# prs-eth/ResDepth

Hardware: AMD Instinct MI355X
Metric: DSM tiles/sec fwd+bwd (256x256, 3-ch, depth-5 U-Net) (higher is better)
Workload: dtype f32

## Files before the change

resdepth_amd/csrc/rd_common.h:

```cpp
#pragma once
#include <hip/hip_runtime.h>
#include <stdint.h>
#include <stdio.h>

#include <tuple>
#include <utility>

#include "../../include/resdepth_hip.h"

namespace rd {

void set_error(const char* fmt, ...);
int check_hip(hipError_t e, const char* what);

struct QuantArgs;
int prof_level();
void prof_begin(hipStream_t s, const char* cls, double flops, double bytes);
void prof_end(hipStream_t s);

struct ProfScope {
    hipStream_t s;
    bool on;
    ProfScope(hipStream_t s_, const char* cls, double flops, double bytes, bool mfma_class = false)
        : s(s_), on(prof_level() >= (mfma_class ? 1 : 2)) {
        if (on) prof_begin(s, cls, flops, bytes);
    }
    ~ProfScope() {
        if (on) prof_end(s);
    }
};

int bn_reduce_finalize(const float* partial, int nb, int c, double count, float eps, float momentum, float* mean, float* invstd,
                       float* rmean, float* rvar, int64_t* nbt, hipStream_t s);
int reduce_partials_f32(const float* partial, double* sums, int nb, int qc, hipStream_t s);

enum TuneKey {
    TUNE_MFMA_F32 = 0,
    TUNE_NT_TILE,
    TUNE_NT_HALO,
    TUNE_NT_SKEW,
    TUNE_TN_TILE,
    TUNE_TN_BLOCKS,
    TUNE_TN_SPLIT,
    TUNE_WG_STRIP,
    TUNE_WG_MINBLOCKS,
    TUNE_WG_BLOCKS,
    TUNE_WG_OCC,
    TUNE_CONVT_PATCH,
    TUNE_EDGE_CONV,
    TUNE_ROWS_BLOCKS,
    TUNE_LAST_BLOCKS,
    TUNE_NT_SPLITK,
    TUNE_NT_EPI,
    TUNE_MFMA_PRODUCTS,
    TUNE_D2H_BLOCKS,
    TUNE_COUNT
};
int tune(int key);
inline int mfma_split() { return !tune(TUNE_MFMA_F32); }
inline int mfma_products() { return tune(TUNE_MFMA_PRODUCTS) == 3 ? 3 : 6; }
struct QuantArgs {
    const unsigned* a;
    const unsigned* b;
    unsigned* out;
    unsigned* out2;
    int img_stride;
};
QuantArgs quant_take();
QuantArgs quant_take_img();
int wgrad_strip_splits(int n, int h, int w, int cin, int cout);
int wgrad_strip_launch(const float* x, const float* dz, float* slab, int n, int h, int w, int cin, int cout, hipStream_t s,
                       int* splits_out, int* swapped_out, const unsigned* x_amax = nullptr, const unsigned* dz_amax = nullptr);

int convt_fwd_launch(const float* x, const void* wsplit, size_t wsplit_bytes, const float* bias, const float* skip,
                     const float* sk_mean, const float* sk_invstd, const float* sk_gamma, const float* sk_beta, float sk_slope,
                     const float* sk_slope_dev, float* out, int n, int h, int w, int cin, int cout, hipStream_t s, int* launched,
                     const QuantArgs& qa);

size_t convt_wgrad_ws_bytes(int n, int h, int w, int cin, int cout);
int convt_wgrad_launch(const float* x, const float* dout, float* slab, int n, int h, int w, int cin, int cout, hipStream_t s,
                       int* splits_out, const unsigned* x_amax = nullptr, const unsigned* dout_amax = nullptr);

int conv_last_fwd_launch(const float* s_in, const float* wt, const float* bias, const float* x_nchw, int xc, float* out, int n,
                         int h, int w, int c, hipStream_t s, int* launched);
int conv_last_dgrad_launch(const float* dout, const float* wt, float* ds, int n, int h, int w, int c, hipStream_t s, int* launched);
int conv_last_dgrad_bn_launch(const float* dout, const float* wt, float* ds, int n, int h, int w, int c, const float* bn_z,
                              const float* mean, const float* invstd, const float* gamma, const float* beta, float slope,
                              const float* slope_dev, float* part, hipStream_t s, int* rows);
int conv_last_wgrad_blocks(int n, int h, int w, int c);
struct TailSkip {
    const float* z;
    const float* mean;
    const float* invstd;
    const float* gamma;
    const float* beta;
    const float* slope_dev;
    float slope;
};
int tail_compose_launch(const float* wt, const float* bt, const float* wl, float* M, float* V, float* VT, float* B9, int cin, int c0,
                        hipStream_t s);
int conv_last_fwd_tail_launch(const TailSkip& sk, const float* t16, const float* b9, const float* wt, const float* bias,
                              const float* x_nchw, int xc, float* out, int n, int h, int w, int c, hipStream_t s);
int conv_last_wgrad_tail_launch(const TailSkip& sk, const float* dout, double* partial, int n, int h, int w, int c, hipStream_t s);
int tail_t16_launch(const TailSkip& sk, const float* V, float* t16, long pixels, int cin, hipStream_t s);
int convt_last_wgrad_launch(const float* x, const TailSkip& sk, const float* dout, const float* wl, float* dwt, double* partial,
                            double* c16, int n, int hc, int wc, int cin, int c0, hipStream_t s);
int conv_last_tail_blocks(int n, int h, int w);
long edge_tiles(int n, int h, int w);
// ... 186 lines not shown
```

resdepth_amd/csrc/rd_elementwise.hip:

```cpp
#include <stdlib.h>

#include "rd_common.h"
#include "rd_mfma_dev.h"

namespace rd {

static inline int grid_cap(long g, int cap) {
    if (g > cap) g = cap;
    if (g < 1) g = 1;
    return (int)g;
}

__device__ __forceinline__ float act_fn(float y, float slope) { return y > 0.f ? y : y * slope; }
__device__ __forceinline__ float act_grad(float y, float slope) { return y > 0.f ? 1.f : slope; }

template <int K>
__device__ __forceinline__ void reduce_rows(double (&vals)[K], double* red, int t, int CQ, int RP, bool active) {
#pragma unroll
    for (int k = 0; k < K; ++k) red[k * 256 + t] = active ? vals[k] : 0.0;
    __syncthreads();
    if (t < CQ) {
#pragma unroll
        for (int k = 0; k < K; ++k) {
            double s = 0.0;
// ... 231 lines not shown
        if (sidx == 2 && dextra) dextra[c] = (float)r;
    }
}

__global__ __launch_bounds__(512) void bn_reduce_finalize_quad_kernel(const float* __restrict__ partial, int nb, int C, double count,
                                                                      float eps, float momentum, float* __restrict__ mean,
                                                                      float* __restrict__ invstd, float* __restrict__ rmean,
                                                                      float* __restrict__ rvar, int64_t* nbt) {
    __shared__ double red[512][4];
    const int t = threadIdx.x, kind = t & 1, slice = t >> 1, cq = blockIdx.x;
    const float* base = partial + (long)kind * C + cq * 4;
    const long stride = 2L * C;
    double a0 = 0.0, a1 = 0.0, a2 = 0.0, a3 = 0.0;
    int b = slice;
    for (; b + 7 * 256 < nb; b += 8 * 256) {
        float4 v[8];
#pragma unroll
        for (int k = 0; k < 8; ++k) v[k] = *reinterpret_cast<const float4*>(base + (long)(b + 256 * k) * stride);
#pragma unroll
        for (int k = 0; k < 8; ++k) {
            a0 += v[k].x; a1 += v[k].y; a2 += v[k].z; a3 += v[k].w;
        }
    }
    for (; b < nb; b += 256) {
        const float4 v = *reinterpret_cast<const float4*>(base + (long)b * stride);
        a0 += v.x; a1 += v.y; a2 += v.z; a3 += v.w;
    }
    red[t][0] = a0; red[t][1] = a1; red[t][2] = a2; red[t][3] = a3;
    __syncthreads();
    for (int sl = 128; sl >= 1; sl >>= 1) {
        if (slice < sl) {
#pragma unroll
            for (int k = 0; k < 4; ++k) red[t][k] += red[t + 2 * sl][k];
        }
        __syncthreads();
    }
    if (t == 0 && blockIdx.x == 0 && nbt) *nbt += 1;
    if (t < 4) {
        const int c = cq * 4 + t;
        const double su = red[0][t], sq = red[1][t];
        const double m = su / count;
        double var = sq / count - m * m;
        if (var < 0.0) var = 0.0;
        mean[c] = (float)m;
        invstd[c] = (float)(1.0 / sqrt(var + (double)eps));
        if (rmean) rmean[c] = (1.f - momentum) * rmean[c] + momentum * (float)m;
        if (rvar) {
            const double unb = count > 1.0 ? var * count / (count - 1.0) : var;
            rvar[c] = (1.f - momentum) * rvar[c] + momentum * (float)unb;
        }
    }
}

int bn_reduce_finalize(const float* partial, int nb, int c, double count, float eps, float momentum, float* mean, float* invstd,
                       float* rmean, float* rvar, int64_t* nbt, hipStream_t s) {
    if (c % 4 == 0)
        RD_LAUNCH(bn_reduce_finalize_quad_kernel, dim3(c / 4), dim3(512), 0, s, partial, nb, c, count, eps, momentum, mean,
                           invstd, rmean, rvar, nbt);
    else
        RD_LAUNCH(bn_reduce_finalize_kernel, dim3(cdiv(c, 4)), dim3(256), 0, s, partial, nb, c, count, eps, momentum, mean,
                           invstd, rmean, rvar, nbt);
    RD_LAUNCH_CHECK("bn_reduce_finalize");
    return RD_OK;
}

__global__ void bn_eval_stats_kernel(const float* __restrict__ rmean, const float* __restrict__ rvar, float eps,
                                     float* __restrict__ mean, float* __restrict__ invstd, int C) {
    const int c = blockIdx.x * blockDim.x + threadIdx.x;
    if (c >= C) return;
    mean[c] = rmean[c];
    invstd[c] = 1.f / sqrtf(rvar[c] + eps);
}

template <bool POOL>
__global__ __launch_bounds__(256) void bn_act_pool_fwd_kernel(const float* __restrict__ z, const float* __restrict__ mean,
                                                              const float* __restrict__ invstd,
                                                              const float* __restrict__ gamma,
                                                              const float* __restrict__ beta, float slope_val,
                                                              const float* __restrict__ slope_dev,
                                                              float* __restrict__ a, float* __restrict__ pooled,
                                                              uint8_t* __restrict__ idx, float* __restrict__ zpool, long rows,
                                                              int H, int W, int C, int CQ, unsigned* a_amax, unsigned* p_amax) {
    const float slope = slope_dev ? slope_dev[0] : slope_val;
    const long total = rows * CQ;
    float amx = 0.f, pmx = 0.f;
    long e0, e1;
    block_range(total, blockIdx.x, gridDim.x, blockDim.x, e0, e1);
    for (long e = e0 + threadIdx.x; e < e1; e += blockDim.x) {
        const int cq = (int)(e % CQ);
        const long row = e / CQ;
        const float4 mu = *reinterpret_cast<const float4*>(mean + cq * 4);
        const float4 is = *reinterpret_cast<const float4*>(invstd + cq * 4);
        const float4 ga = *reinterpret_cast<const float4*>(gamma + cq * 4);
        const float4 be = *reinterpret_cast<const float4*>(beta + cq * 4);
        const float sc[4] = {is.x * ga.x, is.y * ga.y, is.z * ga.z, is.w * ga.w};
        const float sh[4] = {be.x - mu.x * sc[0], be.y - mu.y * sc[1], be.z - mu.z * sc[2], be.w - mu.w * sc[3]};
        if (!POOL) {
            const float4 x = ld_nt4(z + row * C + cq * 4);
            float4 y;
            y.x = act_fn(fmaf(x.x, sc[0], sh[0]), slope);
            y.y = act_fn(fmaf(x.y, sc[1], sh[1]), slope);
            y.z = act_fn(fmaf(x.z, sc[2], sh[2]), slope);
            y.w = act_fn(fmaf(x.w, sc[3], sh[3]), slope);
            *reinterpret_cast<float4*>(a + row * C + cq * 4) = y;
            amx = amax_acc(amax_acc(amax_acc(amax_acc(amx, y.x), y.y), y.z), y.w);
        } else {
            const int W2 = W >> 1, H2 = H >> 1;
            const int j = (int)(row % W2);
            const int i = (int)((row / W2) % H2);
// ... 388 lines not shown
                const float sv[4] = {s4[u].x, s4[u].y, s4[u].z, s4[u].w};
#pragma unroll
                for (int tap = 0; tap < 9; ++tap) {
                    const int dy = tap / 3 - 1, dx = tap % 3 - 1;
                    const int sy = yy - dy, sx = xx - dx;
                    float d = 0.f;
                    if ((unsigned)sy < uH && (unsigned)sx < uW) d = dout[p - dy * W - dx];
#pragma unroll
                    for (int k = 0; k < 4; ++k) acc[tap][k] = fmaf(sv[k], d, acc[tap][k]);
                    if (tap == 4 && cq == 0) accb += d;
                }
            }
        }
    }
    double* out = partial + (long)blockIdx.x * (9 * C + 1);
#pragma unroll
    for (int tap = 0; tap < 9; ++tap) {
        double v[4];
#pragma unroll
        for (int k = 0; k < 4; ++k) v[k] = acc[tap][k];
        reduce_rows<4>(v, red, t, CQ, RP, active);
        if (t < CQ) {
#pragma unroll
            for (int k = 0; k < 4; ++k) out[tap * C + cq * 4 + k] = v[k];
        }
    }
    double vb[4] = {(double)accb, 0.0, 0.0, 0.0};
    reduce_rows<4>(vb, red, t, CQ, RP, active);
    if (t == 0) out[9 * C] = vb[0];
}

__global__ __launch_bounds__(256) void last_wgrad_reduce_kernel(const double* __restrict__ partial,
                                                                float* __restrict__ dw, float* __restrict__ dbias,
                                                                int nb, int C) {
    __shared__ double red[256];
    const int tot = 9 * C + 1;
    const double r = sliced_column_sum<double>(partial, nb, tot, tot, red);
    const int e = blockIdx.x * 16 + threadIdx.x;
    if (threadIdx.x < 16 && e < tot) {
        if (e == 9 * C) {
            if (dbias) dbias[0] = (float)r;
        } else {
            const int tap = e / C, ci = e % C;
            dw[ci * 9 + tap] = (float)r;
        }
    }
}

__device__ __forceinline__ float denorm(float v, float sd, float mu) { return __fadd_rn(__fmul_rn(v, sd), mu); }

__global__ __launch_bounds__(256) void l1_partial_kernel(const float* __restrict__ yp, const float* __restrict__ y,
                                                         const uint8_t* __restrict__ mask, const float* __restrict__ mean,
                                                         const float* __restrict__ stdv, double* __restrict__ partial,
                                                         long total, long pps) {
    __shared__ double red[2 * 256];
    double s = 0.0, c = 0.0;
    for (long e = (long)blockIdx.x * blockDim.x + threadIdx.x; e < total; e += (long)gridDim.x * blockDim.x) {
        if (mask[e]) {
            const int n = (int)(e / pps);
            const float sd = stdv[n], mu = mean[n];
            s += (double)fabsf(denorm(yp[e], sd, mu) - denorm(y[e], sd, mu));
            c += 1.0;
        }
    }
    red[threadIdx.x] = s;
    red[256 + threadIdx.x] = c;
    __syncthreads();
    for (int off = 128; off > 0; off >>= 1) {
        if ((int)threadIdx.x < off) {
            red[threadIdx.x] += red[threadIdx.x + off];
            red[256 + threadIdx.x] += red[256 + threadIdx.x + off];
        }
        __syncthreads();
    }
    if (threadIdx.x == 0) {
        partial[blockIdx.x * 2] = red[0];
        partial[blockIdx.x * 2 + 1] = red[256];
    }
}

__global__ __launch_bounds__(256) void l1_reduce_kernel(const double* __restrict__ partial, double* __restrict__ sums,
                                                        int nb) {
    __shared__ double red[2 * 256];
    double s = 0.0, c = 0.0;
    for (int b = threadIdx.x; b < nb; b += 256) {
        s += partial[b * 2];
        c += partial[b * 2 + 1];
    }
    red[threadIdx.x] = s;
    red[256 + threadIdx.x] = c;
    __syncthreads();
    for (int off = 128; off > 0; off >>= 1) {
        if ((int)threadIdx.x < off) {
            red[threadIdx.x] += red[threadIdx.x + off];
            red[256 + threadIdx.x] += red[256 + threadIdx.x + off];
        }
        __syncthreads();
    }
    if (threadIdx.x == 0) {
        sums[0] = red[0];
        sums[1] = red[256];
    }
}

__global__ __launch_bounds__(256) void l1_finish_kernel(const float* __restrict__ yp, const float* __restrict__ y,
                                                        const uint8_t* __restrict__ mask, const float* __restrict__ mean,
                                                        const float* __restrict__ stdv, const double* __restrict__ sums,
                                                        double numel_total, const float* __restrict__ gout_dev,
                                                        float* __restrict__ loss, float* __restrict__ dyp, long total,
                                                        long pps) {
    const float cnt = (float)sums[1], numel = (float)numel_total;
    const float gout = gout_dev ? gout_dev[0] : 1.f;
    if (blockIdx.x == 0 && threadIdx.x == 0 && loss) {
        float l = (float)(sums[0] / numel_total);
        l = l * numel;
        loss[0] = l / cnt;
    }
    if (!dyp) return;
    const float g = ((gout / cnt) * numel) / numel;
    for (long e = (long)blockIdx.x * blockDim.x + threadIdx.x; e < total; e += (long)gridDim.x * blockDim.x) {
        float o = 0.f;
        if (mask[e]) {
            const int n = (int)(e / pps);
            const float sd = stdv[n], mu = mean[n];
            const float d = denorm(yp[e], sd, mu) - denorm(y[e], sd, mu);
            const float sg = d > 0.f ? 1.f : (d < 0.f ? -1.f : 0.f);
            o = g * sg * sd;
        }
        dyp[e] = o;
    }
// ... 695 lines not shown
    } else {
        ProfScope ps((hipStream_t)s, "bn_act_fwd", 0, 8.0 * pixels * c);
        RD_LAUNCH((bn_act_pool_fwd_kernel<false>), dim3(grid_cap((pixels * CQ + 255) / 256, 8192)), dim3(256),
                           0, (hipStream_t)s, z, mean, invstd, gamma, beta, slope, slope_dev, a, (float*)nullptr,
                           (uint8_t*)nullptr, (float*)nullptr, pixels, h, w, c, CQ, qa.out, (unsigned*)nullptr);
    }
    RD_LAUNCH_CHECK("bn_act_pool_fwd");
    return RD_OK;
}

size_t rd_bn_act_bwd_ws_bytes(int n, int h, int w, int c) {
    RowPlan pl;
    if (!plan_rows((long)n * h * w, c, &pl)) return 0;
    return (size_t)pl.nb * 4 * c * sizeof(double);
}

int rd_bn_act_bwd_reduce(const float* z, const float* mean, const float* invstd, const float* gamma, const float* beta,
                         float slope, const float* slope_dev, const float* g_full, const float* g_pool,
                         const uint8_t* idx, double* sums, float* dgamma, float* dbeta, float* dextra, int n, int h, int w, int c,
                         void* ws, size_t ws_bytes, rd_stream_t s) {
    RD_REQUIRE(z && mean && invstd && gamma && beta && sums, "rd_bn_act_bwd_reduce: null pointer");
    RD_REQUIRE(g_full || g_pool, "rd_bn_act_bwd_reduce: no gradient source");
    RD_REQUIRE(!g_pool || idx, "rd_bn_act_bwd_reduce: g_pool needs idx");
    const bool pool = g_pool != nullptr;
    const long pixels = (long)n * h * w;
    const long rows = pool ? pixels / 4 : pixels;
    RowPlan pl;
    RD_REQUIRE(plan_rows(rows, c, &pl), "rd_bn_act_bwd_reduce: C must be a multiple of 4 and <= 1024 (got %d)", c);
    size_t need = (size_t)pl.nb * 4 * c * sizeof(double);
    if (const size_t q = rd_bn_act_bwd_ws_bytes(n, h, w, c); q > need) need = q;
    if (!ws || ws_bytes < need) {
        set_error("rd_bn_act_bwd_reduce: workspace too small (%zu < %zu)", ws_bytes, need);
        return RD_ERR_WS;
    }
    ProfScope ps((hipStream_t)s, "bn_act_bwd_reduce", 0, 4.0 * pixels * c * (1 + (g_full ? 1 : 0) + (pool ? 0.3 : 0)));
    if (pool)
        RD_LAUNCH((bn_act_bwd_kernel<true, false>), dim3(pl.nb), dim3(256), 0, (hipStream_t)s, z, mean, invstd,
                           gamma, beta, slope, slope_dev, g_full, g_pool, idx, (double*)ws, (const double*)nullptr, 1.0, 1,
                           (float*)nullptr, rows, h, w, c, pl.CQ, pl.RP, pl.rows_per_block, (unsigned*)nullptr);
    else
        RD_LAUNCH((bn_act_bwd_kernel<false, false>), dim3(pl.nb), dim3(256), 0, (hipStream_t)s, z, mean,
                           invstd, gamma, beta, slope, slope_dev, g_full, g_pool, idx, (double*)ws, (const double*)nullptr, 1.0, 1,
                           (float*)nullptr, rows, h, w, c, pl.CQ, pl.RP, pl.rows_per_block, (unsigned*)nullptr);
    RD_LAUNCH(partial_reduce_kernel, dim3(cdiv(4 * c, 16)), dim3(256), 0, (hipStream_t)s, (const double*)ws,
                       sums, pl.nb, 4 * c, c, dbeta, dgamma, dextra);
    RD_LAUNCH_CHECK("bn_act_bwd_reduce");
    return RD_OK;
}

int rd_bn_bwd_stats_finalize(const float* part_a, int rows_a, const float* part_b, int rows_b, int c, double* sums,
                             float* dgamma, float* dbeta, float* dextra, rd_stream_t s) {
    RD_REQUIRE(part_a && rows_a > 0 && sums && c > 0 && c % 4 == 0 && (!part_b || rows_b > 0), "rd_bn_bwd_stats_finalize: bad arguments");
    ProfScope ps((hipStream_t)s, "bn_act_bwd_reduce", 0, 16.0 * c * ((double)rows_a + (part_b ? rows_b : 0)));
    RD_LAUNCH(bn_bwd_stats_finalize_kernel, dim3(c), dim3(256), 0, (hipStream_t)s, part_a, rows_a, part_b,
                       part_b ? rows_b : 0, c, sums, dgamma, dbeta, dextra);
    RD_LAUNCH_CHECK("bn_bwd_stats_finalize");
    return RD_OK;
}

int rd_bn_act_bwd_apply(const float* z, const float* mean, const float* invstd, const float* gamma, const float* beta,
                        float slope, const float* slope_dev, const float* g_full, const float* g_pool,
                        const uint8_t* idx, const double* sums,
                        double count, int training, float* dz, float* dgamma, float* dbeta, int n, int h, int w, int c,
                        rd_stream_t s) {
    RD_REQUIRE(z && mean && invstd && gamma && beta && sums && dz, "rd_bn_act_bwd_apply: null pointer");
    RD_REQUIRE(g_full || g_pool, "rd_bn_act_bwd_apply: no gradient source");
    RD_REQUIRE(!g_pool || idx, "rd_bn_act_bwd_apply: g_pool needs idx");
    RD_REQUIRE(count > 0, "rd_bn_act_bwd_apply: count must be positive");
    const QuantArgs qa = quant_take();
    const bool pool = g_pool != nullptr;
    const long pixels = (long)n * h * w;
    const long rows = pool ? pixels / 4 : pixels;
    RowPlan pl;
    RD_REQUIRE(plan_rows(rows, c, &pl), "rd_bn_act_bwd_apply: C must be a multiple of 4 and <= 1024 (got %d)", c);
    {
        ProfScope ps((hipStream_t)s, "bn_act_bwd_apply", 0,
                     4.0 * pixels * c * (2 + (g_full ? 1 : 0) + (pool ? 0.3 : 0)));
        if (pool)
            RD_LAUNCH((bn_act_bwd_kernel<true, true>), dim3(pl.nb), dim3(256), 0, (hipStream_t)s, z, mean,
                               invstd, gamma, beta, slope, slope_dev, g_full, g_pool, idx, (double*)nullptr, sums, count,
                               training, dz, rows, h, w, c, pl.CQ, pl.RP, pl.rows_per_block, qa.out);
        else
            RD_LAUNCH((bn_act_bwd_kernel<false, true>), dim3(pl.nb), dim3(256), 0, (hipStream_t)s, z, mean,
                               invstd, gamma, beta, slope, slope_dev, g_full, g_pool, idx, (double*)nullptr, sums, count, training,
                               dz, rows, h, w, c, pl.CQ, pl.RP, pl.rows_per_block, qa.out);
    }
    if (dgamma || dbeta)
        RD_LAUNCH(bn_param_grad_kernel, dim3(cdiv(c, 256)), dim3(256), 0, (hipStream_t)s, sums, dgamma, dbeta,
                           c);
    RD_LAUNCH_CHECK("bn_act_bwd_apply");
    return RD_OK;
}

}

static int first_grid(int n, int h, int w, int* tiles_x, int* tiles_y, int* ntiles) {
    *tiles_x = cdiv(w, FT_W);
    *tiles_y = cdiv(h, FT_H);
    *ntiles = n * (*tiles_x) * (*tiles_y);
    return *ntiles < 512 ? *ntiles : 512;
}

template <bool WGRAD>
static int launch_first(const float* x, const float* wt, float* z, const float* dz, float* partial, int n, int h, int w,
                        int cin, int cout, int grid, int tiles_x, int tiles_y, int ntiles, hipStream_t s) {
    const int CQ = cout / 4, PS = 256 / CQ;
#define RD_FIRST_CASE(CI)                                                                                              \
    case CI:                                                                                                           \
// ... 356 lines not shown
    ProfScope ps((hipStream_t)s, "convt_last_wgrad", 2.0 * n * hc * wc * 16.0 * cin, 4.0 * n * hc * wc * (double)(cin + 4));
    const TailSkip sk = {x, mean, invstd, gamma, beta, slope_dev, slope};
    return convt_last_wgrad_launch(x, sk, dout, w_last, dwt_iohw, partial, c16, n, hc, wc, cin, c0, (hipStream_t)s);
}

size_t rd_conv3x3_last_bwd_weight_ws_bytes(int n, int h, int w, int c) {
    if (const int nb = conv_last_wgrad_blocks(n, h, w, c)) return (size_t)nb * (9 * c + 1) * sizeof(double);
    RowPlan pl;
    if (!plan_rows((long)n * h * w, c, &pl, last_blocks())) return 0;
    return (size_t)pl.nb * (9 * c + 1) * sizeof(double);
}

int rd_conv3x3_last_bwd_weight(const float* s_in, const float* dout, float* dw, float* dbias, int n, int h, int w,
                               int c, void* ws, size_t ws_bytes, rd_stream_t s) {
    RD_REQUIRE(s_in && dout && dw, "rd_conv3x3_last_bwd_weight: null pointer");
    RowPlan pl;
    RD_REQUIRE(plan_rows((long)n * h * w, c, &pl, last_blocks()), "rd_conv3x3_last_bwd_weight: C must be a multiple of 4, <= 1024");
    RD_REQUIRE((long)n * h * w < (1L << 31), "rd_conv3x3_last_bwd_weight: pixel count must be < 2^31");
    const size_t need = rd_conv3x3_last_bwd_weight_ws_bytes(n, h, w, c);
    if (!ws || ws_bytes < need) {
        set_error("rd_conv3x3_last_bwd_weight: workspace too small (%zu < %zu)", ws_bytes, need);
        return RD_ERR_WS;
    }
    ProfScope ps((hipStream_t)s, "conv_last_wgrad", 2.0 * n * h * w * 9.0 * c, 4.0 * n * h * w * (double)(c + 1));
    if (const int nb = conv_last_wgrad_blocks(n, h, w, c)) {
        if (int e = conv_last_wgrad_launch(s_in, dout, (double*)ws, n, h, w, c, (hipStream_t)s)) return e;
        RD_LAUNCH(last_wgrad_reduce_kernel, dim3(cdiv(9 * c + 1, 16)), dim3(256), 0, (hipStream_t)s,
                           (const double*)ws, dw, dbias, nb, c);
        RD_LAUNCH_CHECK("conv_last_wgrad");
        return RD_OK;
    }
    RD_LAUNCH(conv_last_wgrad_kernel, dim3(pl.nb), dim3(256), 0, (hipStream_t)s, s_in, dout, (double*)ws,
                       (long)n * h * w, h, w, c, pl.CQ, pl.RP, pl.rows_per_block);
    RD_LAUNCH(last_wgrad_reduce_kernel, dim3(cdiv(9 * c + 1, 16)), dim3(256), 0, (hipStream_t)s,
                       (const double*)ws, dw, dbias, pl.nb, c);
    RD_LAUNCH_CHECK("conv_last_wgrad");
    return RD_OK;
}

static int l1_grid(long total) { return grid_cap((total + 255) / 256, 1024); }

size_t rd_masked_l1_ws_bytes(long long numel) { return (size_t)l1_grid(numel) * 2 * sizeof(double); }

int rd_masked_l1_partial(const float* yp, const float* y, const uint8_t* mask, const float* mean, const float* stdv,
                         double* sums, int n, long long pps, void* ws, size_t ws_bytes, rd_stream_t s) {
    RD_REQUIRE(yp && y && mask && mean && stdv && sums && n > 0 && pps > 0, "rd_masked_l1_partial: bad arguments");
    const long total = (long)n * pps;
    const int nb = l1_grid(total);
    if (!ws || ws_bytes < (size_t)nb * 2 * sizeof(double)) {
        set_error("rd_masked_l1_partial: workspace too small");
        return RD_ERR_WS;
    }
    ProfScope ps((hipStream_t)s, "masked_l1", 0, 9.0 * total);
    RD_LAUNCH(l1_partial_kernel, dim3(nb), dim3(256), 0, (hipStream_t)s, yp, y, mask, mean, stdv, (double*)ws,
                       total, (long)pps);
    RD_LAUNCH(l1_reduce_kernel, dim3(1), dim3(256), 0, (hipStream_t)s, (const double*)ws, sums, nb);
    RD_LAUNCH_CHECK("masked_l1_partial");
    return RD_OK;
}

int rd_masked_l1_finish(const float* yp, const float* y, const uint8_t* mask, const float* mean, const float* stdv,
                        const double* sums, double numel_total, const float* gout, float* loss, float* dyp, int n,
                        long long pps, rd_stream_t s) {
    RD_REQUIRE(yp && y && mask && mean && stdv && sums && n > 0 && pps > 0, "rd_masked_l1_finish: bad arguments");
    const long total = (long)n * pps;
    ProfScope ps((hipStream_t)s, "masked_l1", 0, 13.0 * total);
    RD_LAUNCH(l1_finish_kernel, dim3(dyp ? l1_grid(total) : 1), dim3(256), 0, (hipStream_t)s, yp, y, mask, mean,
                       stdv, sums, numel_total, gout, loss, dyp, total, (long)pps);
    RD_LAUNCH_CHECK("masked_l1_finish");
    return RD_OK;
}

int rd_adam_step(float* p, const float* g, float* m, float* v, long long numel, double beta1, double beta2, float eps,
                 float weight_decay, float step_size, float bc2_sqrt, float grad_scale, rd_stream_t s) {
    RD_REQUIRE(p && g && m && v && numel > 0, "rd_adam_step: bad arguments");
    ProfScope ps((hipStream_t)s, "adam", 0, 28.0 * numel);
    RD_LAUNCH(adam_kernel, dim3(grid_cap((numel + 255) / 256, 8192)), dim3(256), 0, (hipStream_t)s, p, g, m, v,
                       (long)numel, (float)(1.0 - beta1), (float)beta2, (float)(1.0 - beta2), eps, weight_decay, step_size, bc2_sqrt,
                       grad_scale);
    RD_LAUNCH_CHECK("adam");
    return RD_OK;
}

int rd_adam_step_dev(float* p, const float* g, float* m, float* v, long long numel, const float* scalars_dev, rd_stream_t s) {
    RD_REQUIRE(p && g && m && v && scalars_dev && numel > 0, "rd_adam_step_dev: bad arguments");
    ProfScope ps((hipStream_t)s, "adam", 0, 28.0 * numel);
    RD_LAUNCH(adam_dev_kernel, dim3(grid_cap((numel + 255) / 256, 8192)), dim3(256), 0, (hipStream_t)s, p, g, m, v,
                       (long)numel, scalars_dev);
    RD_LAUNCH_CHECK("adam_dev");
    return RD_OK;
}

int rd_sgd_step(float* p, const float* g, float* momentum_buf, long long numel, float lr, float weight_decay, float momentum,
                float dampening, int nesterov, int first_step, float grad_scale, rd_stream_t s) {
    RD_REQUIRE(p && g && numel > 0, "rd_sgd_step: bad arguments");
    RD_REQUIRE(momentum == 0.f || momentum_buf, "rd_sgd_step: momentum != 0 needs a momentum buffer");
    ProfScope ps((hipStream_t)s, "sgd", 0, (momentum != 0.f ? 20.0 : 12.0) * numel);
    const dim3 grid(grid_cap((numel + 255) / 256, 8192));
    if (momentum != 0.f)
        RD_LAUNCH(sgd_kernel<true>, grid, dim3(256), 0, (hipStream_t)s, p, g, momentum_buf, (long)numel, lr, weight_decay,
                           momentum, 1.f - dampening, nesterov, first_step, grad_scale);
    else
        RD_LAUNCH(sgd_kernel<false>, grid, dim3(256), 0, (hipStream_t)s, p, g, (float*)nullptr, (long)numel, lr,
                           weight_decay, 0.f, 1.f, 0, 0, grad_scale);
    RD_LAUNCH_CHECK("sgd");
    return RD_OK;
}

int rd_blend_accumulate(const float* pred, const float* mean, const float* stdv, const int* pos, const int* reg, int n,
// ... 197 lines not shown
```

resdepth_amd/csrc/rd_runtime.hip:

```cpp
#include <hip/hip_ext.h>
#include <stdarg.h>
#include <stdlib.h>
#include <string.h>

#include <mutex>
#include <string>
#include <vector>

#include "rd_common.h"

namespace rd {

static thread_local char g_err[512] = "";

static void quant_clear();
void set_error(const char* fmt, ...) {
    quant_clear();
    va_list ap;
    va_start(ap, fmt);
    vsnprintf(g_err, sizeof(g_err), fmt, ap);
    va_end(ap);
}

int check_hip(hipError_t e, const char* what) {
    if (e == hipSuccess) return RD_OK;
    set_error("%s: %s", what, hipGetErrorString(e));
    return RD_ERR_HIP;
}

struct TuneEntry {
    const char* name;
    int value;
};
static TuneEntry g_tune[TUNE_COUNT] = {
    {"mfma_f32", 0},   {"nt_tile", -1},      {"nt_halo", -1},    {"nt_skew", 1},     {"tn_tile", -1},     {"tn_blocks", 512}, {"tn_split", -1},
    {"wg_strip", -1},  {"wg_minblocks", 768}, {"wg_blocks", 512}, {"wg_occ", 2}, {"convt_patch", -1}, {"edge_conv", -1}, {"rows_blocks", 512}, {"last_blocks", 2048},
    {"nt_splitk", -1}, {"nt_epi", -1}, {"mfma_products", 3}, {"d2h_blocks", 0},
};
static int tune_index(const char* name, size_t len) {
    for (int i = 0; i < TUNE_COUNT; ++i)
        if (strlen(g_tune[i].name) == len && !strncmp(g_tune[i].name, name, len)) return i;
    return -1;
}
static const int g_tune_env = [] {
    if (const char* m = getenv("RD_MFMA"))
    {
        if (!strcmp(m, "f32")) g_tune[TUNE_MFMA_F32].value = 1;
        if (!strcmp(m, "split2h")) g_tune[TUNE_MFMA_PRODUCTS].value = 3;
        if (!strcmp(m, "split3")) g_tune[TUNE_MFMA_PRODUCTS].value = 6;
    }
    const char* e = getenv("RD_TUNE");
    while (e && *e) {
        const char* eq = strchr(e, '=');
        if (!eq) break;
        const int i = tune_index(e, (size_t)(eq - e));
        if (i >= 0) g_tune[i].value = atoi(eq + 1);
        e = strchr(eq, ',');
        if (e) ++e;
    }
    return 0;
}();
int tune(int key) { return g_tune[key].value; }

static thread_local QuantArgs t_quant = {nullptr, nullptr, nullptr, nullptr, 0};
static void quant_clear() { t_quant = {nullptr, nullptr, nullptr, nullptr, 0}; }
QuantArgs quant_take_img() {
    const QuantArgs q = t_quant;
    t_quant = {nullptr, nullptr, nullptr, nullptr, 0};
    return q;
}
QuantArgs quant_take() {
    QuantArgs q = t_quant;
    t_quant = {nullptr, nullptr, nullptr, nullptr, 0};
    if (q.img_stride) q = {nullptr, nullptr, nullptr, nullptr, 0};
    return q;
}

struct PlanOp {
    int kind;
    int role;
    const void* fn;
    dim3 grid, block;
    unsigned shmem;
    int nargs;
    size_t arg0;
    int ev;
};
struct Plan {
    std::vector<PlanOp> ops;
    std::vector<size_t> arg_off;
// ... 102 lines not shown
}

void prof_begin(hipStream_t s, const char* cls, double flops, double bytes) {
    std::lock_guard<std::mutex> lk(g_mu);
    int ci = -1;
    for (size_t i = 0; i < g_cls.size(); ++i)
        if (g_cls[i].name == cls) ci = (int)i;
    if (ci < 0) {
        if (g_cls.size() >= RD_PROF_MAX_CLASSES) return;
        g_cls.push_back(ProfClass());
        g_cls.back().name = cls;
        ci = (int)g_cls.size() - 1;
    }
    ProfRec r;
    r.cls = ci;
    r.e0 = get_event();
    r.e1 = get_event();
    r.flops = flops;
    r.bytes = bytes;
    if (!r.e0 || !r.e1) return;
    (void)hipEventRecord(r.e0, s);
    g_recs.push_back(r);
    t_open = (int)g_recs.size() - 1;
}

void prof_end(hipStream_t s) {
    std::lock_guard<std::mutex> lk(g_mu);
    if (t_open < 0 || t_open >= (int)g_recs.size()) return;
    (void)hipEventRecord(g_recs[t_open].e1, s);
    t_open = -1;
}

static void drain_locked() {
    for (auto& r : g_recs) {
        (void)hipEventSynchronize(r.e1);
        float ms = 0.f;
        if (hipEventElapsedTime(&ms, r.e0, r.e1) == hipSuccess) {
            ProfClass& c = g_cls[r.cls];
            c.launches += 1;
            c.ms += ms;
            c.flops += r.flops;
            c.bytes += r.bytes;
        }
        g_free_events.push_back(r.e0);
        g_free_events.push_back(r.e1);
    }
    g_recs.clear();
}

}

extern "C" {

int rd_version(void) { return 112; }

const char* rd_last_error_string(void) { return rd::g_err; }

int rd_plan_begin(rd_stream_t main_stream, rd_stream_t side_stream) {
    using namespace rd;
    std::lock_guard<std::mutex> lk(g_plan_mu);
    if (g_rec) {
        set_error("rd_plan_begin: a plan is already being recorded");
        return RD_ERR_ARG;
    }
    Plan* p = new Plan();
    p->rec[0] = (hipStream_t)main_stream;
    p->rec[1] = (hipStream_t)side_stream;
    (void)hipGetDevice(&p->dev);
    g_rec = p;
    g_recording = 1;
    return RD_OK;
}

int rd_plan_event_record(rd_stream_t stream) {
    using namespace rd;
    std::lock_guard<std::mutex> lk(g_plan_mu);
    if (!g_rec) return -1;
    const int role = plan_role(g_rec, (hipStream_t)stream);
    if (role < 0) return -1;
    PlanOp op = {};
    op.kind = 1; op.role = role; op.ev = g_rec->n_events++;
    g_rec->ops.push_back(op);
    return op.ev;
}

int rd_plan_event_wait(rd_stream_t stream, int ev) {
    using namespace rd;
    std::lock_guard<std::mutex> lk(g_plan_mu);
    if (!g_rec) return RD_OK;
    const int role = plan_role(g_rec, (hipStream_t)stream);
    if (role < 0 || ev < 0) {
        if (role >= 0 && !g_rec->poisoned) {
            g_rec->poisoned = true;
            g_rec->why = "a plan stream waited for an event recorded outside the plan";
        }
        return RD_OK;
    }
    PlanOp op = {};
    op.kind = 2; op.role = role; op.ev = ev;
    g_rec->ops.push_back(op);
    return RD_OK;
}

int rd_plan_segment(void) {
    using namespace rd;
    std::lock_guard<std::mutex> lk(g_plan_mu);
    if (!g_rec) return -1;
// ... 285 lines not shown
```

Measured before the change: 4514.

## Split BN finalize reductions across blocks with last-block tickets; fuse L1 reduce

Adds multi-block versions of the BatchNorm forward-stats finalize and backward-stats finalize kernels. Each channel quad's partial-sum reduction is spread over 32 or 16 blocks, with partials published to a workspace slab and an atomic ticket electing the last block to combine them. The masked-L1 loss now does its final reduction inside the partial kernel using a two-level ticket scheme, which removes the separate single-block reduce launch. This targets the poor parallelism of one-block-per-channel finalize kernels on large partial counts. In exchange it adds atomic and ticket traffic and depends on shared split-k workspace tickets that must be reset correctly.

```diff
diff --git a/resdepth_amd/csrc/rd_common.h b/resdepth_amd/csrc/rd_common.h
--- a/resdepth_amd/csrc/rd_common.h
+++ b/resdepth_amd/csrc/rd_common.h
@@ -54,6 +54,9 @@
     TUNE_NT_EPI,
     TUNE_MFMA_PRODUCTS,
     TUNE_D2H_BLOCKS,
+    TUNE_BN_FIN_SPLIT,
+    TUNE_BN_BWD_FIN_SPLIT,
+    TUNE_L1_FUSED,
     TUNE_COUNT
 };
 int tune(int key);
diff --git a/resdepth_amd/csrc/rd_elementwise.hip b/resdepth_amd/csrc/rd_elementwise.hip
--- a/resdepth_amd/csrc/rd_elementwise.hip
+++ b/resdepth_amd/csrc/rd_elementwise.hip
@@ -307,9 +307,192 @@
     }
 }
 
+constexpr int kTicketPitch = 32;
+constexpr int kFinTicketLines = 448;
+__device__ __forceinline__ bool last_block_of(unsigned* ticket, unsigned blocks, int* flag) {
+    __atomic_signal_fence(__ATOMIC_SEQ_CST);
+    __builtin_amdgcn_s_waitcnt(0x0F70);
+    __syncthreads();
+    if (threadIdx.x == 0) {
+        const unsigned prev = __hip_atomic_fetch_add(ticket, 1u, __ATOMIC_RELAXED, __HIP_MEMORY_SCOPE_AGENT);
+        *flag = prev == blocks - 1;
+        if (*flag) __hip_atomic_store(ticket, 0u, __ATOMIC_RELAXED, __HIP_MEMORY_SCOPE_AGENT);
+    }
+    __syncthreads();
+    __atomic_signal_fence(__ATOMIC_SEQ_CST);
+    return *flag != 0;
+}
+
+constexpr int kFinBlocks = 32;
+__global__ __launch_bounds__(128) void bn_reduce_finalize_quad_mb_kernel(const float* __restrict__ partial, int nb, int C, double count,
+                                                                         float eps, float momentum, float* __restrict__ mean,
+                                                                         float* __restrict__ invstd, float* __restrict__ rmean,
+                                                                         float* __restrict__ rvar, int64_t* nbt, double* pub,
+                                                                         unsigned* tickets) {
+    __shared__ float4 stage[16][65];
+    __shared__ double red[16][4];
+    __shared__ int last;
+    const int t = threadIdx.x, cq = blockIdx.x / kFinBlocks, r = blockIdx.x - cq * kFinBlocks;
+    const int lp = t & 15, lj = t >> 4;
+    const int lslice = r + 32 * (lp >> 1);
+    const int lrows = lslice < nb ? (nb - lslice + 255) >> 8 : 0;
+    const float* base = partial + (long)(lp & 1) * C + cq * 4 + (long)lslice * 2 * C;
+    const long stride = 512L * C;
+    const int ap = t >> 2, ak = t & 3;
+    const int aslice = r + 32 * (ap >> 1);
+    const int arows = (t < 64 && aslice < nb) ? (nb - aslice + 255) >> 8 : 0;
+    const int rows_max = r < nb ? (nb - r + 255) >> 8 : 0;
+    double acc = 0.0;
+    for (int i0 = 0; i0 < rows_max; i0 += 64) {
+        float4 v[8];
+#pragma unroll
+        for (int k = 0; k < 8; ++k) {
+            const int i = i0 + lj + 8 * k;
+            v[k] = i < lrows ? *reinterpret_cast<const float4*>(base + (long)i * stride) : make_float4(0.f, 0.f, 0.f, 0.f);
+        }
+#pragma unroll
+        for (int k = 0; k < 8; ++k) stage[lp][lj + 8 * k] = v[k];
+        __syncthreads();
+        const int cnt = arows - i0 < 64 ? arows - i0 : 64;
+        for (int i = 0; i < cnt; ++i) acc += reinterpret_cast<const float*>(&stage[ap][i])[ak];
+        __syncthreads();
+    }
+    if (t < 64) red[ap][ak] = acc;
+    __syncthreads();
+    const int kind = (t >> 2) & 1;
+    if (t < 8) {
+        const double l0 = red[0 + kind][ak] + red[8 + kind][ak], l1 = red[2 + kind][ak] + red[10 + kind][ak];
+        const double l2 = red[4 + kind][ak] + red[12 + kind][ak], l3 = red[6 + kind][ak] + red[14 + kind][ak];
+        const double root = (l0 + l2) + (l1 + l3);
+        __hip_atomic_store(pub + (((long)cq * kFinBlocks + r) * 2 + kind) * 4 + ak, root, __ATOMIC_RELAXED, __HIP_MEMORY_SCOPE_AGENT);
+    }
+    if (!last_block_of(tickets + cq * kTicketPitch, kFinBlocks, &last)) return;
+    if (t < 8) {
+        double x[kFinBlocks];
+#pragma unroll
+        for (int i = 0; i < kFinBlocks; ++i)
+            x[i] = __hip_atomic_load(pub + (((long)cq * kFinBlocks + i) * 2 + kind) * 4 + ak, __ATOMIC_RELAXED, __HIP_MEMORY_SCOPE_AGENT);
+#pragma unroll
+        for (int sl = 16; sl >= 1; sl >>= 1)
+#pragma unroll
+            for (int i = 0; i < sl; ++i) x[i] += x[i + sl];
+        red[kind][ak] = x[0];
+    }
+    __syncthreads();
+    if (t == 0 && cq == 0 && nbt) *nbt += 1;
+    if (t < 4) {
+        const int c = cq * 4 + t;
+        const double su = red[0][t], sq = red[1][t];
+        const double m = su / count;
+        double var = sq / count - m * m;
+        if (var < 0.0) var = 0.0;
+        mean[c] = (float)m;
+        invstd[c] = (float)(1.0 / sqrt(var + (double)eps));
+        if (rmean) rmean[c] = (1.f - momentum) * rmean[c] + momentum * (float)m;
+        if (rvar) {
+            const double unb = count > 1.0 ? var * count / (count - 1.0) : var;
+            rvar[c] = (1.f - momentum) * rvar[c] + momentum * (float)unb;
+        }
+    }
+}
+
+constexpr int kBwdFinBlocks = 16;
+__global__ __launch_bounds__(64) void bn_bwd_stats_finalize_mb_kernel(const float* __restrict__ pa, int ra, const float* __restrict__ pb,
+                                                                      int rb, int C, double* __restrict__ sums,
+                                                                      float* __restrict__ dgamma, float* __restrict__ dbeta,
+                                                                      float* __restrict__ dextra, double* pub, unsigned* tickets) {
+    __shared__ int last;
+    const int t = threadIdx.x, sidx = t & 3, sl = t >> 2;
+    const int cq = blockIdx.x / kBwdFinBlocks, j = blockIdx.x - cq * kBwdFinBlocks;
+    const long col = (long)sidx * C + cq * 4, stride = 4L * C;
+    double a0 = 0.0, a1 = 0.0, a2 = 0.0, a3 = 0.0;
+    for (int src = 0; src < 2; ++src) {
+        const float* part = src ? pb : pa;
+        const int nb = src ? rb : ra;
+        if (!part) continue;
+        int b = j * 16 + sl;
+        for (; b + 15 * 256 < nb; b += 16 * 256) {
+            float4 v[16];
+#pragma unroll
+            for (int k = 0; k < 16; ++k) v[k] = *reinterpret_cast<const float4*>(part + (long)(b + 256 * k) * stride + col);
+#pragma unroll
+            for (int k = 0; k < 16; k += 4) {
+                a0 += ((double)v[k].x + (double)v[k + 1].x) + ((double)v[k + 2].x + (double)v[k + 3].x);
+                a1 += ((double)v[k].y + (double)v[k + 1].y) + ((double)v[k + 2].y + (double)v[k + 3].y);
+                a2 += ((double)v[k].z + (double)v[k + 1].z) + ((double)v[k + 2].z + (double)v[k + 3].z);
+                a3 += ((double)v[k].w + (double)v[k + 1].w) + ((double)v[k + 2].w + (double)v[k + 3].w);
+            }
+        }
+        for (; b + 768 < nb; b += 1024) {
+            const float4 v0 = *reinterpret_cast<const float4*>(part + (long)b * stride + col);
+            const float4 v1 = *reinterpret_cast<const float4*>(part + (long)(b + 256) * stride + col);
+            const float4 v2 = *reinterpret_cast<const float4*>(part + (long)(b + 512) * stride + col);
+            const float4 v3 = *reinterpret_cast<const float4*>(part + (long)(b + 768) * stride + col);
+            a0 += ((double)v0.x + (double)v1.x) + ((double)v2.x + (double)v3.x);
+            a1 += ((double)v0.y + (double)v1.y) + ((double)v2.y + (double)v3.y);
+            a2 += ((double)v0.z + (double)v1.z) + ((double)v2.z + (double)v3.z);
+            a3 += ((double)v0.w + (double)v1.w) + ((double)v2.w + (double)v3.w);
+        }
+        for (; b < nb; b += 256) {
+            const float4 v = *reinterpret_cast<const float4*>(part + (long)b * stride + col);
+            a0 += v.x; a1 += v.y; a2 += v.z; a3 += v.w;
+        }
+    }
+#pragma unroll
+    for (int o = 4; o < 64; o <<= 1) {
+        a0 += __shfl_xor(a0, o);
+        a1 += __shfl_xor(a1, o);
+        a2 += __shfl_xor(a2, o);
+        a3 += __shfl_xor(a3, o);
+    }
+    if (t < 4) {
+        double* mine = pub + (((long)cq * kBwdFinBlocks + j) * 4 + sidx) * 4;
+        __hip_atomic_store(mine + 0, a0, __ATOMIC_RELAXED, __HIP_MEMORY_SCOPE_AGENT);
+        __hip_atomic_store(mine + 1, a1, __ATOMIC_RELAXED, __HIP_MEMORY_SCOPE_AGENT);
+        __hip_atomic_store(mine + 2, a2, __ATOMIC_RELAXED, __HIP_MEMORY_SCOPE_AGENT);
+        __hip_atomic_store(mine + 3, a3, __ATOMIC_RELAXED, __HIP_MEMORY_SCOPE_AGENT);
+    }
+    if (!last_block_of(tickets + cq * kTicketPitch, kBwdFinBlocks, &last)) return;
+    if (t < 16) {
+        const int si = t >> 2, k = t & 3;
+        double w[4];
+#pragma unroll
+        for (int wv = 0; wv < 4; ++wv) {
+            double x[4];
+#pragma unroll
+            for (int i = 0; i < 4; ++i)
+                x[i] = __hip_atomic_load(pub + (((long)cq * kBwdFinBlocks + wv * 4 + i) * 4 + si) * 4 + k, __ATOMIC_RELAXED,
+                                         __HIP_MEMORY_SCOPE_AGENT);
+            w[wv] = (x[0] + x[1]) + (x[2] + x[3]);
+        }
+        const double r = ((w[0] + w[1]) + w[2]) + w[3];
+        const int c = cq * 4 + k;
+        sums[(long)si * C + c] = r;
+        if (si == 0 && dbeta) dbeta[c] = (float)r;
+        if (si == 1 && dgamma) dgamma[c] = (float)r;
+        if (si == 2 && dextra) dextra[c] = (float)r;
+    }
+}
+
+static bool finalize_scratch(hipStream_t s, int c, double** pub, unsigned** tickets) {
+    int n_tickets = 0;
+    float* slab = nullptr;
+    size_t slab_bytes = 0;
+    if (!splitk_workspace(s, tickets, &n_tickets, &slab, &slab_bytes)) return false;
+    *pub = reinterpret_cast<double*>(slab);
+    return c / 4 <= kFinTicketLines && (kFinTicketLines + 33) * kTicketPitch <= n_tickets && (size_t)c * 512 <= slab_bytes;
+}
+
 int bn_reduce_finalize(const float* partial, int nb, int c, double count, float eps, float momentum, float* mean, float* invstd,
                        float* rmean, float* rvar, int64_t* nbt, hipStream_t s) {
-    if (c % 4 == 0)
+    const int split = tune(TUNE_BN_FIN_SPLIT);
+    double* pub = nullptr;
+    unsigned* tickets = nullptr;
+    const bool many = split > 0 && (nb >= split || (2L * nb >= split && (long)nb * c >= 128L * split));
+    if (c % 4 == 0 && many && finalize_scratch(s, c, &pub, &tickets))
+        RD_LAUNCH(bn_reduce_finalize_quad_mb_kernel, dim3(c / 4 * kFinBlocks), dim3(128), 0, s, partial, nb, c, count, eps, momentum,
+                           mean, invstd, rmean, rvar, nbt, pub, tickets);
+    else if (c % 4 == 0)
         RD_LAUNCH(bn_reduce_finalize_quad_kernel, dim3(c / 4), dim3(512), 0, s, partial, nb, c, count, eps, momentum, mean,
                            invstd, rmean, rvar, nbt);
     else
@@ -804,8 +987,10 @@
 __global__ __launch_bounds__(256) void l1_partial_kernel(const float* __restrict__ yp, const float* __restrict__ y,
                                                          const uint8_t* __restrict__ mask, const float* __restrict__ mean,
                                                          const float* __restrict__ stdv, double* __restrict__ partial,
-                                                         long total, long pps) {
+                                                         long total, long pps, double* __restrict__ sums,
+                                                         unsigned* ticket) {
     __shared__ double red[2 * 256];
+    __shared__ int last;
     double s = 0.0, c = 0.0;
     for (long e = (long)blockIdx.x * blockDim.x + threadIdx.x; e < total; e += (long)gridDim.x * blockDim.x) {
         if (mask[e]) {
@@ -825,9 +1010,39 @@
         }
         __syncthreads();
     }
+    if (!ticket) {
+        if (threadIdx.x == 0) {
+            partial[blockIdx.x * 2] = red[0];
+            partial[blockIdx.x * 2 + 1] = red[256];
+        }
+        return;
+    }
     if (threadIdx.x == 0) {
-        partial[blockIdx.x * 2] = red[0];
-        partial[blockIdx.x * 2 + 1] = red[256];
+        __hip_atomic_store(partial + blockIdx.x * 2, red[0], __ATOMIC_RELAXED, __HIP_MEMORY_SCOPE_AGENT);
+        __hip_atomic_store(partial + blockIdx.x * 2 + 1, red[256], __ATOMIC_RELAXED, __HIP_MEMORY_SCOPE_AGENT);
+    }
+    const unsigned group = blockIdx.x >> 5, groups = (gridDim.x + 31) >> 5;
+    const unsigned gsize = gridDim.x - group * 32 < 32 ? gridDim.x - group * 32 : 32;
+    if (!last_block_of(ticket + group * kTicketPitch, gsize, &last)) return;
+    if (!last_block_of(ticket + 32 * kTicketPitch, groups, &last)) return;
+    s = c = 0.0;
+    for (int b = threadIdx.x; b < (int)gridDim.x; b += 256) {
+        s += __hip_atomic_load(partial + b * 2, __ATOMIC_RELAXED, __HIP_MEMORY_SCOPE_AGENT);
+        c += __hip_atomic_load(partial + b * 2 + 1, __ATOMIC_RELAXED, __HIP_MEMORY_SCOPE_AGENT);
+    }
+    red[threadIdx.x] = s;
+    red[256 + threadIdx.x] = c;
+    __syncthreads();
+    for (int off = 128; off > 0; off >>= 1) {
+        if ((int)threadIdx.x < off) {
+            red[threadIdx.x] += red[threadIdx.x + off];
+            red[256 + threadIdx.x] += red[256 + threadIdx.x + off];
+        }
+        __syncthreads();
+    }
+    if (threadIdx.x == 0) {
+        sums[0] = red[0];
+        sums[1] = red[256];
     }
 }
 
@@ -1629,8 +1844,16 @@
                              float* dgamma, float* dbeta, float* dextra, rd_stream_t s) {
     RD_REQUIRE(part_a && rows_a > 0 && sums && c > 0 && c % 4 == 0 && (!part_b || rows_b > 0), "rd_bn_bwd_stats_finalize: bad arguments");
     ProfScope ps((hipStream_t)s, "bn_act_bwd_reduce", 0, 16.0 * c * ((double)rows_a + (part_b ? rows_b : 0)));
-    RD_LAUNCH(bn_bwd_stats_finalize_kernel, dim3(c), dim3(256), 0, (hipStream_t)s, part_a, rows_a, part_b,
-                       part_b ? rows_b : 0, c, sums, dgamma, dbeta, dextra);
+    const int split = tune(TUNE_BN_BWD_FIN_SPLIT);
+    const long rows = (long)rows_a + (part_b ? rows_b : 0);
+    double* pub = nullptr;
+    unsigned* tickets = nullptr;
+    if (split > 0 && rows * (c > 32 ? c : 32) >= 64L * split && finalize_scratch((hipStream_t)s, c, &pub, &tickets))
+        RD_LAUNCH(bn_bwd_stats_finalize_mb_kernel, dim3(c / 4 * kBwdFinBlocks), dim3(64), 0, (hipStream_t)s, part_a, rows_a, part_b,
+                           part_b ? rows_b : 0, c, sums, dgamma, dbeta, dextra, pub, tickets);
+    else
+        RD_LAUNCH(bn_bwd_stats_finalize_kernel, dim3(c), dim3(256), 0, (hipStream_t)s, part_a, rows_a, part_b,
+                           part_b ? rows_b : 0, c, sums, dgamma, dbeta, dextra);
     RD_LAUNCH_CHECK("bn_bwd_stats_finalize");
     return RD_OK;
 }
@@ -2093,9 +2316,15 @@
         return RD_ERR_WS;
     }
     ProfScope ps((hipStream_t)s, "masked_l1", 0, 9.0 * total);
+    unsigned* tickets = nullptr;
+    int n_tickets = 0;
+    float* slab = nullptr;
+    size_t slab_bytes = 0;
+    const bool fused = tune(TUNE_L1_FUSED) != 0 && splitk_workspace((hipStream_t)s, &tickets, &n_tickets, &slab, &slab_bytes) &&
+                       (kFinTicketLines + 33) * kTicketPitch <= n_tickets && nb <= 32 * 32;
     RD_LAUNCH(l1_partial_kernel, dim3(nb), dim3(256), 0, (hipStream_t)s, yp, y, mask, mean, stdv, (double*)ws,
-                       total, (long)pps);
-    RD_LAUNCH(l1_reduce_kernel, dim3(1), dim3(256), 0, (hipStream_t)s, (const double*)ws, sums, nb);
+                       total, (long)pps, sums, fused ? tickets + kFinTicketLines * kTicketPitch : (unsigned*)nullptr);
+    if (!fused) RD_LAUNCH(l1_reduce_kernel, dim3(1), dim3(256), 0, (hipStream_t)s, (const double*)ws, sums, nb);
     RD_LAUNCH_CHECK("masked_l1_partial");
     return RD_OK;
 }
diff --git a/resdepth_amd/csrc/rd_runtime.hip b/resdepth_amd/csrc/rd_runtime.hip
--- a/resdepth_amd/csrc/rd_runtime.hip
+++ b/resdepth_amd/csrc/rd_runtime.hip
@@ -36,6 +36,7 @@
     {"mfma_f32", 0},   {"nt_tile", -1},      {"nt_halo", -1},    {"nt_skew", 1},     {"tn_tile", -1},     {"tn_blocks", 512}, {"tn_split", -1},
     {"wg_strip", -1},  {"wg_minblocks", 768}, {"wg_blocks", 512}, {"wg_occ", 2}, {"convt_patch", -1}, {"edge_conv", -1}, {"rows_blocks", 512}, {"last_blocks", 2048},
     {"nt_splitk", -1}, {"nt_epi", -1}, {"mfma_products", 3}, {"d2h_blocks", 0},
+    {"bn_fin_split", 4096}, {"bn_bwd_fin_split", 5120}, {"l1_fused", 1},
 };
 static int tune_index(const char* name, size_t len) {
     for (int i = 0; i < TUNE_COUNT; ++i)
@@ -244,7 +245,7 @@
 
 extern "C" {
 
-int rd_version(void) { return 112; }
+int rd_version(void) { return 113; }
 
 const char* rd_last_error_string(void) { return rd::g_err; }
 
```

Result: no change. 4545 (median of 6 runs) (+0.7%).
